# Keytoyze/Mug-Diffusion

Measured on NVIDIA H100. Metric: denoising-steps/sec, higher is better.
Workload: dtype f32

## Files before the change

### include/mugd.h

```cpp
#ifndef MUGD_H
#define MUGD_H

#include <stdint.h>

#ifdef __cplusplus
extern "C" {
#endif

#define MUGD_ABI_VERSION 13

typedef struct mugd_handle mugd_handle;
typedef struct mugd_plan mugd_plan;

enum mugd_status {
    MUGD_OK = 0,
    MUGD_ERR_INVALID = 1,
    MUGD_ERR_CUDA = 2,
    MUGD_ERR_NO_DEVICE = 3,
    MUGD_ERR_OOM = 4
};

enum mugd_op_kind {
    MUGD_OP_GEMM = 1,
    MUGD_OP_GROUPNORM = 2,
// ... 275 lines not shown

int  mugd_remove_mini_jacks(mugd_handle* h, const int32_t* chart_start, int32_t n_charts, double jack_interval,
                            const double* start, const double* end, const uint8_t* is_long, int32_t* x, uint8_t* state,
                            void* workspace, void* stream);

int  mugd_gemm_tc_query(mugd_handle* h, const mugd_gemm* g, int32_t sm_count, int32_t* supported, int32_t* splits,
                        int64_t* workspace_bytes, int32_t* n_tiles);
int  mugd_gemm_tc_variant(const mugd_gemm* g, int32_t sm_count, int32_t* tile_n, int32_t* ctas_per_sm, int32_t* grid_ctas);

int  mugd_set_tc_single_pass_tf32(mugd_handle* h, int enabled);

int  mugd_set_attention_impl(mugd_handle* h, int impl);

int  mugd_set_s4conv_impl(mugd_handle* h, int impl);

int  mugd_debug_set_tc_cost(float kstep128_us, float kstep256_us, float split_us, float two_cta_fixed_us);

int  mugd_debug_set_tc_tile_n(int bn);

int  mugd_debug_set_attention_dump(float* buf);

int  mugd_debug_set_tc_timing(long long* device_buf);

int  mugd_fill_i32(int32_t* dst, int32_t value, void* stream);
int  mugd_abi_sizes(int32_t* out, int32_t n);

#ifdef __cplusplus
}
#endif
#endif
// ... 1 lines not shown
```

### mug_diffusion_b200/csrc/api.cu

```cuda
#include <stdarg.h>
#include <string.h>

#include <vector>

#include "common.cuh"

namespace mugd {

static thread_local char g_err[1024] = "";
bool g_use_pdl = true;

void set_error(const char* fmt, ...) {
    va_list ap;
    va_start(ap, fmt);
    vsnprintf(g_err, sizeof(g_err), fmt, ap);
    va_end(ap);
}

}

struct mugd_handle {
    mugd::DeviceInfo dev;
    int default_gemm_impl = MUGD_GEMM_SIMT;
};
// ... 36 lines not shown
static int run_steps(const mugd_plan* eval_plan, int32_t n_steps, int32_t* step, cudaStream_t st, Before before, After after) {
    mugd_step_advance adv;
    adv.step = step;
    for (int32_t k = 0; k < n_steps; ++k) {
        int rc = before(k);
        if (rc != MUGD_OK) return rc;
        MUGD_CHECK_CUDA(cudaGraphLaunch(eval_plan->exec, st));
        if ((rc = after(k)) != MUGD_OK) return rc;
        if (step && (rc = launch_step_advance(eval_plan->h->dev, adv, st, nullptr)) != MUGD_OK) return rc;
    }
    return MUGD_OK;
}

static int no_kernels(int32_t) { return MUGD_OK; }

template <typename Before>
static int run_tail_steps(const mugd_plan* eval_plan, const mugd_op* tail, int32_t n_tail, int32_t n_steps, cudaStream_t st,
                          Before before) {
    return run_steps(eval_plan, n_steps, nullptr, st, before, [&](int32_t) {
        for (int32_t k = 0; k < n_tail; ++k) {
            int rc = dispatch(eval_plan->h, tail[k], st, nullptr);
            if (rc != MUGD_OK) return rc;
        }
        return (int)MUGD_OK;
    });
}

static int run_dpm_steps(const mugd_plan* eval_plan, const mugd_dpm_ex& e, int32_t n_steps, cudaStream_t st) {
    return run_steps(
        eval_plan, n_steps, e.dpm.step, st, [&](int32_t k) { return e.stage ? launch_stage(*e.stage, k, st) : MUGD_OK; },
// ... 80 lines not shown
}

int mugd_set_attention_impl(mugd_handle* h, int impl) {
    MUGD_REQUIRE(h, "null handle");
    h->dev.attention_impl = impl ? 1 : 0;
    return MUGD_OK;
}

int mugd_set_s4conv_impl(mugd_handle* h, int impl) {
    MUGD_REQUIRE(h, "null handle");
    MUGD_REQUIRE(impl >= 0 && impl <= 2, "set_s4conv_impl: %d (0 = automatic, 1 = resident, 2 = streamed)", impl);
    h->dev.s4conv_impl = impl;
    return MUGD_OK;
}

int mugd_set_pdl(int enabled) {
    g_use_pdl = enabled != 0;
    return MUGD_OK;
}

int mugd_op_run(mugd_handle* h, const mugd_op* op, void* stream) {
    MUGD_REQUIRE(h && op, "mugd_op_run: null argument");
    return dispatch(h, *op, (cudaStream_t)stream, nullptr);
}

int mugd_plan_create(mugd_handle* h, const mugd_op* ops, int32_t n_ops, mugd_plan** out) {
    MUGD_REQUIRE(h && ops && out && n_ops > 0, "mugd_plan_create: bad arguments");
    mugd_plan* p = new mugd_plan();
    p->h = h;
    p->ops.assign(ops, ops + n_ops);
    *out = p;
    return MUGD_OK;
}

int mugd_plan_run(mugd_plan* p, void* stream) {
    MUGD_REQUIRE(p, "null plan");
    int launches = 0;
    const size_t n = p->ops.size();
    std::vector<const mugd_gemm*> next_tc(n, nullptr);
    for (size_t i = n; i-- > 1;) {
        const mugd_op& o = p->ops[i];
        next_tc[i - 1] = o.kind == MUGD_OP_GEMM && gemm_runs_tc(o.u.gemm, p->h->default_gemm_impl) ? &o.u.gemm : next_tc[i];
    }
    for (size_t i = 0; i < n; ++i) {
        int rc = dispatch(p->h, p->ops[i], (cudaStream_t)stream, &launches, next_tc[i]);
        if (rc != MUGD_OK) {
            char prev[900];
            strncpy(prev, g_err, sizeof(prev) - 1);
            prev[sizeof(prev) - 1] = 0;
            set_error("plan op %zu (kind %d, tag %d): %s", i, p->ops[i].kind, p->ops[i].tag, prev);
            return rc;
        }
    }
    p->launches = launches;
    return MUGD_OK;
}

int mugd_plan_capture(mugd_plan* p, void* stream) {
    MUGD_REQUIRE(p, "null plan");
    cudaStream_t st = (cudaStream_t)stream;
// ... 161 lines not shown
```

### mug_diffusion_b200/csrc/common.cuh

```cuda
#pragma once
#include <cuda_runtime.h>
#include <stdint.h>
#include <stdio.h>
#include <string.h>
#include <string>
#include <utility>

#include "../../include/mugd.h"

#if defined(__CUDA_ARCH__) && (__CUDA_ARCH__ != 900)
#error "libmugd is written for sm_90a (H100) only"
#endif

namespace mugd {

void set_error(const char* fmt, ...);

#define MUGD_CHECK_CUDA(expr)                                                             \
    do {                                                                                  \
        cudaError_t _e = (expr);                                                          \
        if (_e != cudaSuccess) {                                                          \
            ::mugd::set_error("%s:%d %s -> %s", __FILE__, __LINE__, #expr,                \
                              cudaGetErrorString(_e));                                    \
            return MUGD_ERR_CUDA;                                                         \
// ... 4 lines not shown
    do {                                                                                  \
        if (!(cond)) {                                                                    \
            ::mugd::set_error(__VA_ARGS__);                                               \
            return MUGD_ERR_INVALID;                                                      \
        }                                                                                 \
    } while (0)

struct DeviceInfo {
    int device = 0;
    int sm_count = 132;
    int cc_major = 0, cc_minor = 0;
    int max_smem_optin = 0;
    int tc_single_pass = 0;
    int attention_impl = 1;
    int s4conv_impl = 0;
};

int launch_gemm(const DeviceInfo& dev, const mugd_gemm& g, int default_impl, const mugd_gemm* next, cudaStream_t st, int* launches);
bool gemm_runs_tc(const mugd_gemm& g, int default_impl);
int launch_groupnorm(const DeviceInfo& dev, const mugd_groupnorm& g, cudaStream_t st, int* launches);
int launch_layernorm(const DeviceInfo& dev, const mugd_layernorm& g, cudaStream_t st, int* launches);
int launch_attention(const DeviceInfo& dev, const mugd_attention& a, cudaStream_t st, int* launches);
int launch_s4conv(const DeviceInfo& dev, const mugd_s4conv& s, cudaStream_t st, int* launches);
int launch_ddim_update(const DeviceInfo& dev, const mugd_ddim_update& d, cudaStream_t st, int* launches);
int launch_transpose(const DeviceInfo& dev, const mugd_transpose& t, cudaStream_t st, int* launches);
int launch_copy2d(const DeviceInfo& dev, const mugd_copy2d& c, cudaStream_t st, int* launches);
int launch_step_advance(const DeviceInfo& dev, const mugd_step_advance& a, cudaStream_t st, int* launches);
int launch_notes(const DeviceInfo& dev, const mugd_notes& n, cudaStream_t st, int* launches);
int launch_embed(const DeviceInfo& dev, const mugd_embed& e, cudaStream_t st, int* launches);
int launch_tf32_split(const DeviceInfo& dev, const mugd_tf32_split& s, cudaStream_t st, int* launches);
int launch_posterior(const DeviceInfo& dev, const mugd_posterior& p, cudaStream_t st, int* launches);
int check_stage(const mugd_stage& s, int32_t n_steps);
int launch_stage(const mugd_stage& s, int32_t i, cudaStream_t st);
int check_plms(const mugd_plms& p);
int launch_plms_combine(const mugd_plms& p, int32_t step, int heun, cudaStream_t st);
int check_ddpm(const mugd_ddpm& d);
int launch_ddpm_update(const mugd_ddpm& d, int32_t k, cudaStream_t st);
int check_dpm(const mugd_dpm& d);
int launch_dpm_update(const mugd_dpm& d, cudaStream_t st);
int check_dpm_ex(const mugd_dpm_ex& e, int32_t n_steps);
int launch_dpm_ex_update(const mugd_dpm_ex& e, cudaStream_t st);
int check_join(const mugd_join& j);
int launch_join(const mugd_join& j, const int32_t* step, cudaStream_t st);
int launch_gemm_tc(const DeviceInfo& dev, const mugd_gemm& g, const mugd_gemm* next, cudaStream_t st, int* launches);
bool gemm_tc_supported(const mugd_gemm& g);

inline int check_cfg(const char* who, int cfg) {
    MUGD_REQUIRE(cfg == 0 || cfg == 1, "%s: cfg=%d", who, cfg);
    return MUGD_OK;
}
inline int check_scale(const char* who, float scale) {
    MUGD_REQUIRE(isfinite(scale), "%s: scale is not finite", who);
    return MUGD_OK;
}
inline int check_x_dup(const char* who, const float* x_dup, int cfg) {
    MUGD_REQUIRE(!x_dup == !cfg, "%s: x_dup must be given exactly when cfg = 1 (the evaluation reads x in both halves)", who);
    return MUGD_OK;
}
inline int check_tile_grid(const char* who, int32_t B, int32_t C, int32_t L) {
// ... 74 lines not shown
```

### mug_diffusion_b200/csrc/gemm_simt.cu

```cuda
#include "common.cuh"

namespace mugd {

constexpr int SG_THREADS = 256;
constexpr int SG_BK = 16;

struct GemmParams {
    mugd_gemm g;
    int nk;
};

__device__ __forceinline__ int conv_src_row(int mode, int l, int t, int Lin, int Lout, int tap_shift, int dil) {
    if (mode == MUGD_CONV_NONE) return l;
    if (mode == MUGD_CONV_SAME) {
        const int r = l + t - 1;
        return (r >= 0 && r < Lin) ? r : -1;
    }
    if (mode == MUGD_CONV_DOWN) {
        const int r = 2 * l + t;
        return (r < Lin) ? r : -1;
    }
    if (mode == MUGD_CONV_TAPS) {
        const int r = l + (t + tap_shift) * dil;
        return (r >= 0 && r < Lin) ? r : -1;
// ... 192 lines not shown
    MUGD_REQUIRE(aligned16(g.A) && aligned16(g.W) && g.lda % 4 == 0 && g.lda >= g.K, "gemm: A/W alignment or lda");
    MUGD_REQUIRE(!g.bias || aligned16(g.bias), "gemm: bias alignment");
    MUGD_REQUIRE(!g.rowvec || (aligned16(g.rowvec) && g.rowvec_b_stride % 4 == 0 && g.rowvec_step_stride % 4 == 0), "gemm: rowvec alignment");
    const int nout = g.gate == MUGD_GATE_NONE ? g.N : g.N / 2;
    const int al = g.gate == MUGD_GATE_NONE ? 4 : 2;
    MUGD_REQUIRE(g.ldc >= nout && g.ldc % al == 0 && (reinterpret_cast<uintptr_t>(g.C) % (4 * al)) == 0, "gemm: C alignment/ldc");
    MUGD_REQUIRE(!g.residual || (g.ldr >= nout && g.ldr % al == 0 && (reinterpret_cast<uintptr_t>(g.residual) % (4 * al)) == 0), "gemm: residual alignment/ldr");
    MUGD_REQUIRE(g.act >= 0 && g.act <= 2 && g.gate >= 0 && g.gate <= 2, "gemm: bad act/gate");
    return MUGD_OK;
}

bool gemm_runs_tc(const mugd_gemm& g, int default_impl) {
    return (g.impl == MUGD_GEMM_AUTO ? default_impl : g.impl) == MUGD_GEMM_TC && gemm_tc_supported(g);
}

int launch_gemm(const DeviceInfo& dev, const mugd_gemm& g, int default_impl, const mugd_gemm* next, cudaStream_t st, int* launches) {
    int rc = validate_gemm(g);
    if (rc != MUGD_OK) return rc;
    int impl = g.impl == MUGD_GEMM_AUTO ? default_impl : g.impl;
    if (impl == MUGD_GEMM_TC) {
        if (gemm_tc_supported(g)) return launch_gemm_tc(dev, g, next, st, launches);
        MUGD_REQUIRE(g.impl != MUGD_GEMM_TC, "gemm: tensor-core path requested but shape unsupported (M=%d N=%d K=%d)", g.M, g.N, g.K);
    }
    MUGD_REQUIRE(!(g.W_hi && g.W_hi == g.W), "gemm: W was split into TF32 hi/lo in place, the FFMA kernel needs the plain fp32 weight (M=%d N=%d K=%d)", g.M, g.N, g.K);
    MUGD_REQUIRE(!g.row_moments && !g.ln_stats,
                 "gemm: the row-moment sink / folded LayerNorm exist on the tensor-core path only (M=%d N=%d K=%d fell to the FFMA kernel)", g.M, g.N, g.K);
    GemmParams p;
    p.g = g;
    p.nk = (g.taps * g.K + g.K2) / SG_BK;
    const long tiles128 = (long)((g.M + 127) / 128) * ((g.N + 127) / 128);
    if (tiles128 >= 2L * dev.sm_count) {
        dim3 grid((g.N + 127) / 128, (g.M + 127) / 128);
        MUGD_CHECK_CUDA(launch_k(gemm_simt_kernel<2, 2>, grid, dim3(SG_THREADS), 0, st, p));
    } else {
        dim3 grid((g.N + 63) / 64, (g.M + 63) / 64);
        MUGD_CHECK_CUDA(launch_k(gemm_simt_kernel<1, 1>, grid, dim3(SG_THREADS), 0, st, p));
// ... 8 lines not shown
```

### mug_diffusion_b200/csrc/gemm_tc.cu

```cuda
#include "gemm_tc.cuh"

namespace mugd {

template <int BN, int EPI>
__global__ void __launch_bounds__(TC_THREADS, 1)
gemm_tc_kernel(const __grid_constant__ CUtensorMap tmA, const __grid_constant__ CUtensorMap tmA1,
               const __grid_constant__ CUtensorMap tmA2, const __grid_constant__ CUtensorMap tmB, const __grid_constant__ CUtensorMap tmWhi,
               const __grid_constant__ CUtensorMap tmWlo, const __grid_constant__ TcParams p) {
    extern __shared__ uint8_t smem_raw[];
    const uint32_t base = (smem_u32(smem_raw) + 1023u) & ~1023u;
    const TcBars<BN> B(base);
    TC_STAMP(p, 0, blockIdx.x == 0 && blockIdx.y == 0 && blockIdx.z == 0);
    if (threadIdx.x < 32) {
        B.init_parallel((int)threadIdx.x);
    } else if (threadIdx.x < 38) {
        const CUtensorMap* m = threadIdx.x == 32 ? &tmA : threadIdx.x == 33 ? &tmA1 : threadIdx.x == 34 ? &tmA2
                             : threadIdx.x == 35 ? &tmB : threadIdx.x == 36 ? &tmWhi : &tmWlo;
        asm volatile("prefetch.tensormap [%0];" ::"l"(reinterpret_cast<uint64_t>(m)) : "memory");
    }
    __syncthreads();
    TC_STAMP(p, 1, blockIdx.x == 0 && blockIdx.y == 0 && blockIdx.z == 0);
    gemm_tc_tile<BN, EPI>(&tmA, &tmA1, &tmA2, &tmB, &tmWhi, &tmWlo, p, blockIdx.x, blockIdx.y, blockIdx.z, base);
}

// ... 140 lines not shown
    p.ws = (float*)g.workspace;
    p.gy = t.gy;
    p.ln_invK = 1.0 / (double)g.K;
    if (next) {
        p.pf_hi = next->W_hi;
        p.pf_lo = p.hot.single_pass ? nullptr : next->W_lo;
        p.pf_bytes = (int64_t)next->N * ((int64_t)next->taps * next->K + next->K2) * 4;
    }
#ifdef MUGD_TC_TIMELINE
    p.dbg = g_tc_dbg;
#endif
    out->BN = t.BN;
    return MUGD_OK;
}

template <int BN, int EPI>
static int tc_launch(const TcPlanned& pl, cudaStream_t st) {
    const TcParams& p = pl.p;
    const TcParams::Hot& h = p.hot;
    if (h.splits > 1) {
        MUGD_CHECK_CUDA(launch_k(gemm_tc_kernel<BN, TC_E_NONE>, dim3(h.gx, p.gy, h.splits), dim3(TC_THREADS), TcSmem<BN>::TOTAL, st, pl.maps[0],
                                 pl.maps[1], pl.maps[2], pl.maps[3], pl.maps[4], pl.maps[5], p));
        MUGD_CHECK_CUDA(launch_k(gemm_tc_reduce_kernel<BN, EPI>, dim3((unsigned)(h.gx * p.gy * (TC_BM / TC_RED_ROWS<BN>))), dim3(TC_THREADS), 0,
                                 st, p));
        return MUGD_OK;
    }
    MUGD_CHECK_CUDA(launch_k(gemm_tc_kernel<BN, EPI>, dim3(h.gx, p.gy, 1), dim3(TC_THREADS), TcSmem<BN>::TOTAL, st, pl.maps[0], pl.maps[1],
                             pl.maps[2], pl.maps[3], pl.maps[4], pl.maps[5], p));
    return MUGD_OK;
}

template <int BN, int... EPI>
static cudaError_t allow_smem_bn(int bytes, std::integer_sequence<int, EPI...>) {
    return allow_dynamic_smem(bytes, gemm_tc_kernel<BN, EPI>...);
}
cudaError_t gemm_tc_allow_smem(int bytes) {
    const cudaError_t e = allow_smem_bn<64>(bytes, std::make_integer_sequence<int, TC_E_COUNT>{});
// ... 2 lines not shown

template <int BN>
static int tc_launch_bn(const TcPlanned& pl, cudaStream_t st) {
    switch (tc_epi_of(pl.p.g)) {
        case TC_E_GEGLU: return tc_launch<BN, TC_E_GEGLU>(pl, st);
        case TC_E_GLU: return tc_launch<BN, TC_E_GLU>(pl, st);
        case TC_E_SILU: return tc_launch<BN, TC_E_SILU>(pl, st);
        case TC_E_GELU: return tc_launch<BN, TC_E_GELU>(pl, st);
        case TC_E_SINK: return tc_launch<BN, TC_E_SINK>(pl, st);
        case TC_E_LN: return tc_launch<BN, TC_E_LN>(pl, st);
        case TC_E_LN_GEGLU: return tc_launch<BN, TC_E_LN_GEGLU>(pl, st);
        default: return tc_launch<BN, TC_E_NONE>(pl, st);
    }
}

int launch_gemm_tc(const DeviceInfo& dev, const mugd_gemm& g, const mugd_gemm* next, cudaStream_t st, int* launches) {
    TcPlanned pl;
    int rc = tc_plan(dev, g, next, &pl);
    if (rc != MUGD_OK) return rc;
    if (pl.BN == 128) rc = tc_launch_bn<128>(pl, st);
    else rc = tc_launch_bn<64>(pl, st);
    if (rc != MUGD_OK) return rc;
    if (launches) *launches += pl.p.hot.splits > 1 ? 2 : 1;
    return MUGD_OK;
}

}

extern "C" int mugd_debug_set_tc_cost(float kstep128_us, float kstep256_us, float split_us, float two_cta_fixed_us) {
    (void)kstep256_us;
    (void)two_cta_fixed_us;
    if (kstep128_us > 0.f) mugd::g_tc_kstep128 = kstep128_us;
    if (split_us > 0.f) mugd::g_tc_split = split_us;
    return MUGD_OK;
// ... 54 lines not shown
```

### mug_diffusion_b200/csrc/gemm_tc.cuh

```cuda
#pragma once
#include <cuda.h>
#include <stddef.h>

#include <type_traits>

#include "common.cuh"
#include "wgmma.cuh"

namespace mugd {

constexpr int TC_BM = 128;
constexpr int TC_BK = 32;
constexpr int TC_THREADS = 256;
constexpr uint32_t TC_A_BYTES = TC_BM * TC_BK * 4;

struct TcParams {
    struct Hot {
        int32_t Lrows, Bs;
        int32_t box_l, box_b;
        int32_t tiles_per_sample;
        int32_t it_base, it_rem;
        int32_t it_main;
        int32_t kblocks;
        int32_t total_it;
        int32_t splits;
        int32_t single_pass;
        int32_t conv_mode, tap_shift, tap_dilation;
        int32_t gx;
    } hot;
    mugd_gemm g;
    float* ws;
    int32_t gy;
    double ln_invK;
    const float* pf_hi;
    const float* pf_lo;
    int64_t pf_bytes;
#ifdef MUGD_TC_TIMELINE
    long long* dbg;
#endif
};
static_assert(sizeof(TcParams::Hot) == 64 && offsetof(TcParams, hot) == 0, "the hot fields are the first 64 bytes of the parameters");

#ifdef __CUDACC__
__device__ __forceinline__ long long gtimer() {
    long long t;
    asm volatile("mov.u64 %0, %%globaltimer;" : "=l"(t) :: "memory");
    return t;
}
#ifdef MUGD_TC_TIMELINE
#define TC_STAMP(p, k, cta0) do { if ((p).dbg && (cta0) && threadIdx.x == 0) (p).dbg[k] = gtimer(); } while (0)
#else
// ... 151 lines not shown
}

__device__ __forceinline__ void tc_tile_rows(const TcParams& p, int by, int& b_base, int& l_base, int& rows_valid) {
    const TcParams::Hot& h = p.hot;
    if (h.Lrows >= TC_BM) {
        b_base = by / h.tiles_per_sample;
        l_base = (by % h.tiles_per_sample) * TC_BM;
        rows_valid = min(TC_BM, h.Lrows - l_base);
    } else {
        b_base = by * h.box_b;
        l_base = 0;
        rows_valid = min(h.box_b, h.Bs - b_base) * h.Lrows;
    }
}

template <int BN>
struct TcBars {
    using S = TcSmem<BN>;
    static constexpr int COUNT = 2 * S::STAGES;
    static_assert(8 * COUNT <= (int)S::BAR_BYTES, "barrier block");
    uint32_t bars;
    __device__ __forceinline__ explicit TcBars(uint32_t base) : bars(base + S::TILE_BYTES) {}
    __device__ __forceinline__ uint32_t full(int s) const { return bars + 8u * s; }
    __device__ __forceinline__ uint32_t empty(int s) const { return bars + 8u * (S::STAGES + s); }
    __device__ __forceinline__ void init_parallel(int t) const {
        if (t >= COUNT) return;
        mbar_init(bars + 8u * t, t < S::STAGES ? 1u : (uint32_t)(TC_THREADS / 32));
        mbar_init_fence();
    }
};
// ... 172 lines not shown
    __syncthreads();
    TC_STAMP(p, 3, bx == 0 && by == 0 && bz == 0);
    {
        const float* rowvec = g.rowvec ? g.rowvec + (int64_t)epi_step * g.rowvec_step_stride : nullptr;
        if (h.splits > 1) {
            const int tile_lin = by * h.gx + bx;
            float* wsp = p.ws + ((int64_t)tile_lin * h.splits + bz) * (TC_BM * BN);
            constexpr int C4 = BN / 4;
            constexpr int U = 8;
#pragma unroll 1
            for (int i0 = 0; i0 < TC_BM * C4; i0 += TC_THREADS * U) {
                float4 a4[U];
#pragma unroll
                for (int u = 0; u < U; ++u) {
                    const int idx = i0 + u * TC_THREADS + (int)threadIdx.x;
                    const int row = idx / C4, c4 = idx - row * C4;
                    a4[u] = lds_f4(base + (uint32_t)(row * SP + c4 * 4) * 4u);
                }
#pragma unroll
                for (int u = 0; u < U; ++u) st_f4(wsp + (i0 + u * TC_THREADS + (int)threadIdx.x) * 4, a4[u]);
            }
        } else {
            using E = TcEpiTraits<EPI>;
            tc_store_tile<BN, E::ACT, E::GATE, E::MODE>(g, base, m_base, n0, rows_valid, rowvec, base + S::TILE_BYTES - 1024u, epi_bias, epi_cs);
        }
    }
    TC_STAMP(p, 4, bx == 0 && by == 0 && bz == 0);
}

template <int BN> constexpr int TC_RED_ROWS = TC_THREADS / (BN / 4);

// ... 73 lines not shown
```

### mug_diffusion_b200/csrc/norm.cu

```cuda
#include "common.cuh"

namespace mugd {

constexpr int GN_THREADS = 256;
constexpr int GN_MAXV = 32;

__device__ __forceinline__ void gn_block_stats(double s, double ss, double inv_n, float eps, float& mean, float& rstd) {
    __shared__ double red[2][GN_THREADS / 32];
    s = warp_sum(s);
    ss = warp_sum(ss);
    const int warp = threadIdx.x >> 5, lane = threadIdx.x & 31;
    if (lane == 0) { red[0][warp] = s; red[1][warp] = ss; }
    __syncthreads();
    double ts = 0.0, tss = 0.0;
#pragma unroll
    for (int w = 0; w < GN_THREADS / 32; ++w) { ts += red[0][w]; tss += red[1][w]; }
    const double m = ts * inv_n;
    const double var = tss * inv_n - m * m;
    const float v = fmaxf((float)var, 0.f) + eps;
    float r = rsqrtf(v);
    r = r * (1.5f - 0.5f * v * r * r);
    mean = (float)m;
    rstd = r;
}

template <int NV>
__global__ void __launch_bounds__(GN_THREADS)
groupnorm_silu_reg_kernel(const float* __restrict__ x, int64_t ldx, float* __restrict__ y, int64_t ldy,
                          const float* __restrict__ gamma, const float* __restrict__ beta,
                          int L, int C, int G, float eps, int silu) {
    pdl_wait();
    const int g = blockIdx.x, b = blockIdx.y;
    const int cg = C / G;
    const int q = cg >> 2;
    const int total = L * q;
    const double inv_n = 1.0 / ((double)L * cg);
    const float* xb = x + (int64_t)b * L * ldx + (int64_t)g * cg;
    float* yb = y + (int64_t)b * L * ldy + (int64_t)g * cg;
    float4 v[NV];
#pragma unroll
    for (int u = 0; u < NV; ++u) {
        const int i = (int)threadIdx.x + u * GN_THREADS;
        v[u] = make_float4(0.f, 0.f, 0.f, 0.f);
        if (i < total) {
            const int row = i / q, qq = i - row * q;
            v[u] = ld_f4(xb + (int64_t)row * ldx + qq * 4);
        }
    }
    double s = 0.0, ss = 0.0;
#pragma unroll
    for (int u = 0; u < NV; ++u) {
        s += (double)v[u].x + (double)v[u].y + (double)v[u].z + (double)v[u].w;
        ss += (double)v[u].x * v[u].x + (double)v[u].y * v[u].y + (double)v[u].z * v[u].z + (double)v[u].w * v[u].w;
    }
    const float* gm = gamma + g * cg;
    const float* bt = beta + g * cg;
    constexpr bool PRE = NV <= 8;
    float4 gav[PRE ? NV : 1], bev[PRE ? NV : 1];
    if constexpr (PRE) {
#pragma unroll
        for (int u = 0; u < NV; ++u) {
            const int i = (int)threadIdx.x + u * GN_THREADS;
            const int qq = i < total ? i % q : 0;
            gav[u] = ld_f4(gm + qq * 4);
            bev[u] = ld_f4(bt + qq * 4);
        }
    }
    float mean, rstd;
    gn_block_stats(s, ss, inv_n, eps, mean, rstd);
#pragma unroll
    for (int u = 0; u < NV; ++u) {
        const int i = (int)threadIdx.x + u * GN_THREADS;
        if (i < total) {
            const int row = i / q, qq = i - row * q;
            float4 ga, be;
            if constexpr (PRE) { ga = gav[u]; be = bev[u]; }
            else { ga = ld_f4(gm + qq * 4); be = ld_f4(bt + qq * 4); }
            float4 o;
            o.x = (v[u].x - mean) * rstd * ga.x + be.x;
            o.y = (v[u].y - mean) * rstd * ga.y + be.y;
            o.z = (v[u].z - mean) * rstd * ga.z + be.z;
            o.w = (v[u].w - mean) * rstd * ga.w + be.w;
            if (silu) { o.x = silu_f(o.x); o.y = silu_f(o.y); o.z = silu_f(o.z); o.w = silu_f(o.w); }
            st_f4(yb + (int64_t)row * ldy + qq * 4, o);
        }
    }
}

__global__ void __launch_bounds__(GN_THREADS)
groupnorm_silu_kernel(const float* __restrict__ x, int64_t ldx, float* __restrict__ y, int64_t ldy,
                      const float* __restrict__ gamma, const float* __restrict__ beta,
                      int L, int C, int G, float eps, int silu) {
    pdl_wait();
    const int g = blockIdx.x, b = blockIdx.y;
    const int cg = C / G;
    const int q = cg >> 2;
    const int total = L * q;
    const double inv_n = 1.0 / ((double)L * cg);
    const float* xb = x + (int64_t)b * L * ldx + (int64_t)g * cg;
    float* yb = y + (int64_t)b * L * ldy + (int64_t)g * cg;

// ... 11 lines not shown
    for (int i = threadIdx.x; i < total; i += GN_THREADS) {
        const int row = i / q, qq = i - row * q;
        const float4 v = ld_f4(xb + (int64_t)row * ldx + qq * 4);
        const float4 ga = ld_f4(gm + qq * 4);
        const float4 be = ld_f4(bt + qq * 4);
        float4 o;
        o.x = (v.x - mean) * rstd * ga.x + be.x;
        o.y = (v.y - mean) * rstd * ga.y + be.y;
        o.z = (v.z - mean) * rstd * ga.z + be.z;
        o.w = (v.w - mean) * rstd * ga.w + be.w;
        if (silu) { o.x = silu_f(o.x); o.y = silu_f(o.y); o.z = silu_f(o.z); o.w = silu_f(o.w); }
        st_f4(yb + (int64_t)row * ldy + qq * 4, o);
    }
}

int launch_groupnorm(const DeviceInfo&, const mugd_groupnorm& g, cudaStream_t st, int* launches) {
    MUGD_REQUIRE(g.B > 0 && g.L > 0 && g.C > 0 && g.G > 0, "groupnorm: empty shape B=%d L=%d C=%d G=%d", g.B, g.L, g.C, g.G);
    MUGD_REQUIRE(g.C % g.G == 0 && (g.C / g.G) % 4 == 0, "groupnorm: C/G must be a multiple of 4 (C=%d G=%d)", g.C, g.G);
    MUGD_REQUIRE(g.ldx % 4 == 0 && g.ldy % 4 == 0 && aligned16(g.x) && aligned16(g.y) && aligned16(g.gamma) && aligned16(g.beta),
                 "groupnorm: operands must be 16-byte aligned with ld %% 4 == 0");
    MUGD_REQUIRE(g.ldx >= g.C && g.ldy >= g.C, "groupnorm: leading dimension smaller than C");
    dim3 grid(g.G, g.B);
    const int per_thread = (g.L * (g.C / g.G / 4) + GN_THREADS - 1) / GN_THREADS;
#define GN_GO(K) MUGD_CHECK_CUDA(launch_k(K, grid, dim3(GN_THREADS), 0, st, g.x, g.ldx, g.y, g.ldy, g.gamma, g.beta, g.L, g.C, g.G, g.eps, g.silu))
    if (per_thread <= 2) GN_GO(groupnorm_silu_reg_kernel<2>);
    else if (per_thread <= 4) GN_GO(groupnorm_silu_reg_kernel<4>);
    else if (per_thread <= 8) GN_GO(groupnorm_silu_reg_kernel<8>);
    else if (per_thread <= 16) GN_GO(groupnorm_silu_reg_kernel<16>);
    else if (per_thread <= GN_MAXV) GN_GO(groupnorm_silu_reg_kernel<GN_MAXV>);
    else GN_GO(groupnorm_silu_kernel);
#undef GN_GO
    if (launches) *launches += 1;
    return MUGD_OK;
}

constexpr int LN_WARPS = 8;
constexpr int LN_MAXQ = 8;

// ... 62 lines not shown
```

### mug_diffusion_b200/lib.py

```python
from __future__ import annotations

import ctypes as C
import os
from typing import Optional

HERE = os.path.dirname(os.path.abspath(__file__))
LIB_PATH = os.environ.get("MUGD_LIB") or os.path.join(HERE, "libmugd.so")

(OP_GEMM, OP_GROUPNORM, OP_LAYERNORM, OP_ATTENTION, OP_S4CONV, OP_DDIM_UPDATE, OP_TRANSPOSE, OP_COPY2D, OP_STEP_ADVANCE, OP_NOTES, OP_EMBED,
 OP_TF32_SPLIT, OP_POSTERIOR) = range(1, 14)
CONV_NONE, CONV_SAME, CONV_DOWN, CONV_UP, CONV_TAPS = range(5)
ACT_NONE, ACT_SILU, ACT_GELU = range(3)
GATE_NONE, GATE_GEGLU, GATE_GLU = range(3)
GEMM_AUTO, GEMM_SIMT, GEMM_TC = range(3)
ABI_VERSION = 13

_f = C.c_void_p


class Gemm(C.Structure):
    _fields_ = [("A", _f), ("lda", C.c_int64), ("W", _f), ("W_hi", _f), ("W_lo", _f), ("bias", _f), ("rowvec", _f),
                ("rowvec_b_stride", C.c_int64), ("rowvec_step_stride", C.c_int64), ("step", _f),
                ("residual", _f), ("ldr", C.c_int64), ("C", _f), ("ldc", C.c_int64),
                ("M", C.c_int32), ("N", C.c_int32), ("K", C.c_int32),
# ... 186 lines not shown
    lib.mugd_sample_plms.argtypes = [C.c_void_p, C.POINTER(Plms), C.c_int32, C.c_int32, C.c_void_p]
    lib.mugd_plms_combine.argtypes = [C.POINTER(Plms), C.c_int32, C.c_int32, C.c_void_p]
    lib.mugd_sample_ddpm.argtypes = [C.c_void_p, C.POINTER(Ddpm), C.c_int32, C.c_int32, C.c_void_p]
    lib.mugd_ddpm_update.argtypes = [C.POINTER(Ddpm), C.c_void_p]
    lib.mugd_sample_dpm.argtypes = [C.c_void_p, C.POINTER(Dpm), C.c_int32, C.c_int32, C.c_void_p]
    lib.mugd_dpm_update.argtypes = [C.POINTER(Dpm), C.c_void_p]
    lib.mugd_sample_dpm_ex.argtypes = [C.c_void_p, C.POINTER(DpmEx), C.c_int32, C.c_int32, C.c_void_p]
    lib.mugd_dpm_ex_update.argtypes = [C.POINTER(DpmEx), C.c_void_p]
    lib.mugd_stochastic_encode.argtypes = [C.POINTER(QEncode), C.c_void_p]
    lib.mugd_sample_join.argtypes = [C.c_void_p, C.POINTER(Join), C.POINTER(Op), C.c_int32, C.c_int32, C.c_int32, C.c_void_p]
    lib.mugd_plan_save.argtypes = [C.c_void_p, C.POINTER(Region), C.c_int32, C.c_char_p]
    lib.mugd_plan_load.argtypes = [C.c_void_p, C.c_char_p, C.POINTER(Region), C.c_int32, C.POINTER(C.c_void_p)]
    lib.mugd_set_tc_single_pass_tf32.argtypes = [C.c_void_p, C.c_int]
    lib.mugd_set_attention_impl.argtypes = [C.c_void_p, C.c_int]
    lib.mugd_set_s4conv_impl.argtypes = [C.c_void_p, C.c_int]
    lib.mugd_debug_set_tc_tile_n.argtypes = [C.c_int]
    lib.mugd_debug_set_tc_cost.argtypes = [C.c_float, C.c_float, C.c_float, C.c_float]
    if os.environ.get("MUGD_TC_COST"):
        lib.mugd_debug_set_tc_cost(*([float(v) for v in os.environ["MUGD_TC_COST"].split(",")] + [0.0] * 4)[:4])
    if os.environ.get("MUGD_TC_TILE"):
        lib.mugd_debug_set_tc_tile_n(int(os.environ["MUGD_TC_TILE"]))
    if os.environ.get("MUGD_TC_BN"):
        lib.mugd_debug_set_tc_tile_n(int(os.environ["MUGD_TC_BN"]))
    if os.environ.get("MUGD_PDL") in ("0", "1"):
        lib.mugd_set_pdl(int(os.environ["MUGD_PDL"]))
    _lib = lib
    return lib


def check(rc: int, what: str = ""):
    if rc != 0:
        msg = load().mugd_last_error().decode(errors="replace")
        if rc == 4:
            import torch
            raise torch.cuda.OutOfMemoryError(f"{what}: {msg}")
        raise MugdError(f"{what} failed (status {rc}): {msg}")


EXPORTED_SYMBOLS = [
    "mugd_abi_version", "mugd_last_error", "mugd_create", "mugd_destroy", "mugd_device_info", "mugd_set_gemm_impl",
    "mugd_op_run", "mugd_plan_create", "mugd_plan_run", "mugd_plan_capture", "mugd_plan_replay",
    "mugd_plan_launch_count", "mugd_plan_destroy", "mugd_s4_kernel_gen", "mugd_fill_i32", "mugd_abi_sizes", "mugd_gemm_tc_query",
    "mugd_set_pdl", "mugd_set_tc_single_pass_tf32", "mugd_set_attention_impl", "mugd_set_s4conv_impl", "mugd_debug_set_tc_tile_n", "mugd_debug_set_tc_cost", "mugd_gemm_tc_variant",
    "mugd_debug_set_attention_dump", "mugd_debug_set_tc_timing", "mugd_sample", "mugd_plan_save", "mugd_plan_load", "mugd_plan_regions", "mugd_plan_ops",
    "mugd_melspec", "mugd_grid_scan", "mugd_chart_snap", "mugd_remove_mini_jacks",
    "mugd_sample_staged", "mugd_sample_plms", "mugd_plms_combine",
    "mugd_sample_ddpm", "mugd_ddpm_update", "mugd_stochastic_encode", "mugd_sample_join",
    "mugd_sample_dpm", "mugd_dpm_update", "mugd_sample_dpm_ex", "mugd_dpm_ex_update",
]
```

Before: 244.0.

## Fuse split-K GEMM reduction into following GroupNorm kernel

When a split-K tensor-core GEMM with a plain epilogue is immediately followed by a GroupNorm over its output, the GEMM now launches only its partial-product kernel. The GroupNorm kernel then sums the split-K partials from the workspace, applies the GEMM finish (bias, residual, row vector, store of C) and normalizes in the same pass. This drops one kernel launch and one write-then-read round trip of the GEMM output per matched pair. The workspace layout switches to quad-major for these pairs so the GroupNorm reads line up. The cost is per-group blocks that each reduce many splits, which can leave the GPU with lower parallelism than the dedicated reduce kernel had. The path is on by default and can be disabled.

Result: faster. 248.1, median of 6 (+1.7%).

```diff
diff --git a/include/mugd.h b/include/mugd.h
--- a/include/mugd.h
+++ b/include/mugd.h
@@ -313,6 +313,9 @@
 
 int  mugd_set_s4conv_impl(mugd_handle* h, int impl);
 
+int  mugd_set_gn_reduce_fusion(mugd_handle* h, int enabled);
+int  mugd_gn_reduce_pairs(const mugd_op* ops, int32_t n_ops, int32_t sm_count, int32_t* paired, int32_t* n_pairs);
+
 int  mugd_debug_set_tc_cost(float kstep128_us, float kstep256_us, float split_us, float two_cta_fixed_us);
 
 int  mugd_debug_set_tc_tile_n(int bn);
diff --git a/mug_diffusion_b200/csrc/api.cu b/mug_diffusion_b200/csrc/api.cu
--- a/mug_diffusion_b200/csrc/api.cu
+++ b/mug_diffusion_b200/csrc/api.cu
@@ -4,6 +4,7 @@
 #include <vector>
 
 #include "common.cuh"
+#include "gemm_tc.cuh"
 
 namespace mugd {
 
@@ -74,6 +75,11 @@
 
 static int no_kernels(int32_t) { return MUGD_OK; }
 
+static bool gn_finishes_op(const mugd_op* op, size_t n, int default_impl, int sm_count) {
+    return n >= 2 && op[0].kind == MUGD_OP_GEMM && op[1].kind == MUGD_OP_GROUPNORM &&
+           gn_finishes_gemm(op[0].u.gemm, op[1].u.gn, default_impl, sm_count);
+}
+
 template <typename Before>
 static int run_tail_steps(const mugd_plan* eval_plan, const mugd_op* tail, int32_t n_tail, int32_t n_steps, cudaStream_t st,
                           Before before) {
@@ -184,6 +190,30 @@
     return MUGD_OK;
 }
 
+int mugd_set_gn_reduce_fusion(mugd_handle* h, int enabled) {
+    MUGD_REQUIRE(h, "null handle");
+    MUGD_REQUIRE(enabled == 0 || enabled == 1, "set_gn_reduce_fusion: %d (0 = reduce launch, 1 = the GroupNorm finishes the GEMM)", enabled);
+    h->dev.gn_reduce_fusion = enabled;
+    return MUGD_OK;
+}
+
+int mugd_gn_reduce_pairs(const mugd_op* ops, int32_t n_ops, int32_t sm_count, int32_t* paired, int32_t* n_pairs) {
+    MUGD_REQUIRE(ops && n_ops > 0, "gn_reduce_pairs: bad arguments");
+    const int sms = sm_count > 0 ? sm_count : 132;
+    int32_t count = 0;
+    for (int32_t i = 0; i < n_ops; ++i) {
+        const bool pair = gn_finishes_op(ops + i, (size_t)(n_ops - i), MUGD_GEMM_TC, sms);
+        if (paired) paired[i] = pair ? 1 : 0;
+        if (pair) {
+            ++count;
+            if (paired) paired[i + 1] = 0;
+            ++i;
+        }
+    }
+    if (n_pairs) *n_pairs = count;
+    return MUGD_OK;
+}
+
 int mugd_set_pdl(int enabled) {
     g_use_pdl = enabled != 0;
     return MUGD_OK;
@@ -207,13 +237,22 @@
     MUGD_REQUIRE(p, "null plan");
     int launches = 0;
     const size_t n = p->ops.size();
+    const mugd_handle* h = p->h;
     std::vector<const mugd_gemm*> next_tc(n, nullptr);
     for (size_t i = n; i-- > 1;) {
         const mugd_op& o = p->ops[i];
-        next_tc[i - 1] = o.kind == MUGD_OP_GEMM && gemm_runs_tc(o.u.gemm, p->h->default_gemm_impl) ? &o.u.gemm : next_tc[i];
-    }
+        next_tc[i - 1] = o.kind == MUGD_OP_GEMM && gemm_runs_tc(o.u.gemm, h->default_gemm_impl) ? &o.u.gemm : next_tc[i];
+    }
+    const cudaStream_t st = (cudaStream_t)stream;
     for (size_t i = 0; i < n; ++i) {
-        int rc = dispatch(p->h, p->ops[i], (cudaStream_t)stream, &launches, next_tc[i]);
+        int rc;
+        if (h->dev.gn_reduce_fusion && gn_finishes_op(p->ops.data() + i, n - i, h->default_gemm_impl, h->dev.sm_count)) {
+            TcPlanned pl;
+            rc = launch_gemm(h->dev, p->ops[i].u.gemm, h->default_gemm_impl, next_tc[i], st, &launches, &pl);
+            if (rc == MUGD_OK) rc = launch_groupnorm(h->dev, p->ops[++i].u.gn, st, &launches, &pl);
+        } else {
+            rc = dispatch(p->h, p->ops[i], st, &launches, next_tc[i]);
+        }
         if (rc != MUGD_OK) {
             char prev[900];
             strncpy(prev, g_err, sizeof(prev) - 1);
diff --git a/mug_diffusion_b200/csrc/common.cuh b/mug_diffusion_b200/csrc/common.cuh
--- a/mug_diffusion_b200/csrc/common.cuh
+++ b/mug_diffusion_b200/csrc/common.cuh
@@ -42,11 +42,16 @@
     int tc_single_pass = 0;
     int attention_impl = 1;
     int s4conv_impl = 0;
+    int gn_reduce_fusion = 1;
 };
 
-int launch_gemm(const DeviceInfo& dev, const mugd_gemm& g, int default_impl, const mugd_gemm* next, cudaStream_t st, int* launches);
+struct TcPlanned;
+
+int launch_gemm(const DeviceInfo& dev, const mugd_gemm& g, int default_impl, const mugd_gemm* next, cudaStream_t st, int* launches,
+                TcPlanned* partials = nullptr);
 bool gemm_runs_tc(const mugd_gemm& g, int default_impl);
-int launch_groupnorm(const DeviceInfo& dev, const mugd_groupnorm& g, cudaStream_t st, int* launches);
+bool gn_finishes_gemm(const mugd_gemm& g, const mugd_groupnorm& n, int default_impl, int sm_count);
+int launch_groupnorm(const DeviceInfo& dev, const mugd_groupnorm& g, cudaStream_t st, int* launches, const TcPlanned* partials = nullptr);
 int launch_layernorm(const DeviceInfo& dev, const mugd_layernorm& g, cudaStream_t st, int* launches);
 int launch_attention(const DeviceInfo& dev, const mugd_attention& a, cudaStream_t st, int* launches);
 int launch_s4conv(const DeviceInfo& dev, const mugd_s4conv& s, cudaStream_t st, int* launches);
@@ -70,7 +75,7 @@
 int launch_dpm_ex_update(const mugd_dpm_ex& e, cudaStream_t st);
 int check_join(const mugd_join& j);
 int launch_join(const mugd_join& j, const int32_t* step, cudaStream_t st);
-int launch_gemm_tc(const DeviceInfo& dev, const mugd_gemm& g, const mugd_gemm* next, cudaStream_t st, int* launches);
+int launch_gemm_tc(const DeviceInfo& dev, const mugd_gemm& g, const mugd_gemm* next, cudaStream_t st, int* launches, TcPlanned* partials);
 bool gemm_tc_supported(const mugd_gemm& g);
 
 inline int check_cfg(const char* who, int cfg) {
diff --git a/mug_diffusion_b200/csrc/gemm_simt.cu b/mug_diffusion_b200/csrc/gemm_simt.cu
--- a/mug_diffusion_b200/csrc/gemm_simt.cu
+++ b/mug_diffusion_b200/csrc/gemm_simt.cu
@@ -230,12 +230,14 @@
     return (g.impl == MUGD_GEMM_AUTO ? default_impl : g.impl) == MUGD_GEMM_TC && gemm_tc_supported(g);
 }
 
-int launch_gemm(const DeviceInfo& dev, const mugd_gemm& g, int default_impl, const mugd_gemm* next, cudaStream_t st, int* launches) {
+int launch_gemm(const DeviceInfo& dev, const mugd_gemm& g, int default_impl, const mugd_gemm* next, cudaStream_t st, int* launches,
+                TcPlanned* partials) {
     int rc = validate_gemm(g);
     if (rc != MUGD_OK) return rc;
     int impl = g.impl == MUGD_GEMM_AUTO ? default_impl : g.impl;
+    MUGD_REQUIRE(!partials || (impl == MUGD_GEMM_TC && gemm_tc_supported(g)), "gemm: only the tensor-core kernel can leave split-K partials");
     if (impl == MUGD_GEMM_TC) {
-        if (gemm_tc_supported(g)) return launch_gemm_tc(dev, g, next, st, launches);
+        if (gemm_tc_supported(g)) return launch_gemm_tc(dev, g, next, st, launches, partials);
         MUGD_REQUIRE(g.impl != MUGD_GEMM_TC, "gemm: tensor-core path requested but shape unsupported (M=%d N=%d K=%d)", g.M, g.N, g.K);
     }
     MUGD_REQUIRE(!(g.W_hi && g.W_hi == g.W), "gemm: W was split into TF32 hi/lo in place, the FFMA kernel needs the plain fp32 weight (M=%d N=%d K=%d)", g.M, g.N, g.K);
diff --git a/mug_diffusion_b200/csrc/gemm_tc.cu b/mug_diffusion_b200/csrc/gemm_tc.cu
--- a/mug_diffusion_b200/csrc/gemm_tc.cu
+++ b/mug_diffusion_b200/csrc/gemm_tc.cu
@@ -178,13 +178,21 @@
     return MUGD_OK;
 }
 
+template <int BN>
+static int tc_launch_partials(const TcPlanned& pl, cudaStream_t st) {
+    const TcParams& p = pl.p;
+    MUGD_CHECK_CUDA(launch_k(gemm_tc_kernel<BN, TC_E_NONE>, dim3(p.hot.gx, p.gy, p.hot.splits), dim3(TC_THREADS), TcSmem<BN>::TOTAL, st,
+                             pl.maps[0], pl.maps[1], pl.maps[2], pl.maps[3], pl.maps[4], pl.maps[5], p));
+    return MUGD_OK;
+}
+
 template <int BN, int EPI>
 static int tc_launch(const TcPlanned& pl, cudaStream_t st) {
     const TcParams& p = pl.p;
     const TcParams::Hot& h = p.hot;
     if (h.splits > 1) {
-        MUGD_CHECK_CUDA(launch_k(gemm_tc_kernel<BN, TC_E_NONE>, dim3(h.gx, p.gy, h.splits), dim3(TC_THREADS), TcSmem<BN>::TOTAL, st, pl.maps[0],
-                                 pl.maps[1], pl.maps[2], pl.maps[3], pl.maps[4], pl.maps[5], p));
+        int rc = tc_launch_partials<BN>(pl, st);
+        if (rc != MUGD_OK) return rc;
         MUGD_CHECK_CUDA(launch_k(gemm_tc_reduce_kernel<BN, EPI>, dim3((unsigned)(h.gx * p.gy * (TC_BM / TC_RED_ROWS<BN>))), dim3(TC_THREADS), 0,
                                  st, p));
         return MUGD_OK;
@@ -217,10 +225,19 @@
     }
 }
 
-int launch_gemm_tc(const DeviceInfo& dev, const mugd_gemm& g, const mugd_gemm* next, cudaStream_t st, int* launches) {
-    TcPlanned pl;
+int launch_gemm_tc(const DeviceInfo& dev, const mugd_gemm& g, const mugd_gemm* next, cudaStream_t st, int* launches, TcPlanned* partials) {
+    TcPlanned local;
+    TcPlanned& pl = partials ? *partials : local;
     int rc = tc_plan(dev, g, next, &pl);
     if (rc != MUGD_OK) return rc;
+    if (partials) {
+        MUGD_REQUIRE(pl.p.hot.splits > 1 && tc_epi_of(g) == TC_E_NONE, "gemm_tc: only a split-K GEMM with a plain epilogue can leave its partials");
+        pl.p.ws_quad_major = 1;
+        rc = pl.BN == 128 ? tc_launch_partials<128>(pl, st) : tc_launch_partials<64>(pl, st);
+        if (rc != MUGD_OK) return rc;
+        if (launches) *launches += 1;
+        return MUGD_OK;
+    }
     if (pl.BN == 128) rc = tc_launch_bn<128>(pl, st);
     else rc = tc_launch_bn<64>(pl, st);
     if (rc != MUGD_OK) return rc;
diff --git a/mug_diffusion_b200/csrc/gemm_tc.cuh b/mug_diffusion_b200/csrc/gemm_tc.cuh
--- a/mug_diffusion_b200/csrc/gemm_tc.cuh
+++ b/mug_diffusion_b200/csrc/gemm_tc.cuh
@@ -35,6 +35,7 @@
     const float* pf_hi;
     const float* pf_lo;
     int64_t pf_bytes;
+    int32_t ws_quad_major;
 #ifdef MUGD_TC_TIMELINE
     long long* dbg;
 #endif
@@ -216,6 +217,17 @@
     }
 }
 
+__device__ __forceinline__ int64_t tc_ws_offset(const TcParams& p, int bn, int m, int n) {
+    const TcParams::Hot& h = p.hot;
+    const int s = m / h.Lrows, l = m - s * h.Lrows;
+    int by, r;
+    if (h.Lrows >= TC_BM) { by = s * h.tiles_per_sample + l / TC_BM; r = l % TC_BM; }
+    else { by = s / h.box_b; r = m - by * h.box_b * h.Lrows; }
+    const int bx = n / bn, c = n - bx * bn;
+    const int64_t in_tile = p.ws_quad_major ? (int64_t)(c >> 2) * (TC_BM * 4) + r * 4 + (c & 3) : (int64_t)r * bn + c;
+    return ((int64_t)(by * h.gx + bx) * h.splits) * (TC_BM * bn) + in_tile;
+}
+
 template <int BN>
 struct TcBars {
     using S = TcSmem<BN>;
@@ -418,7 +430,9 @@
 #pragma unroll
                 for (int u = 0; u < U; ++u) {
                     const int idx = i0 + u * TC_THREADS + (int)threadIdx.x;
-                    const int row = idx / C4, c4 = idx - row * C4;
+                    int row, c4;
+                    if (p.ws_quad_major) { c4 = idx / TC_BM; row = idx - c4 * TC_BM; }
+                    else { row = idx / C4; c4 = idx - row * C4; }
                     a4[u] = lds_f4(base + (uint32_t)(row * SP + c4 * 4) * 4u);
                 }
 #pragma unroll
diff --git a/mug_diffusion_b200/csrc/norm.cu b/mug_diffusion_b200/csrc/norm.cu
--- a/mug_diffusion_b200/csrc/norm.cu
+++ b/mug_diffusion_b200/csrc/norm.cu
@@ -1,9 +1,11 @@
 #include "common.cuh"
+#include "gemm_tc.cuh"
 
 namespace mugd {
 
 constexpr int GN_THREADS = 256;
 constexpr int GN_MAXV = 32;
+constexpr int GN_REDUCE_MAXV = 2;
 
 __device__ __forceinline__ void gn_block_stats(double s, double ss, double inv_n, float eps, float& mean, float& rstd) {
     __shared__ double red[2][GN_THREADS / 32];
@@ -22,6 +24,47 @@
     r = r * (1.5f - 0.5f * v * r * r);
     mean = (float)m;
     rstd = r;
+}
+
+template <int NV>
+__device__ __forceinline__ void gn_normalize_slab(const float4 (&v)[NV], float* yb, int64_t ldy, const float* gm, const float* bt, int q,
+                                                  int total, double inv_n, float eps, int silu) {
+    double s = 0.0, ss = 0.0;
+#pragma unroll
+    for (int u = 0; u < NV; ++u) {
+        s += (double)v[u].x + (double)v[u].y + (double)v[u].z + (double)v[u].w;
+        ss += (double)v[u].x * v[u].x + (double)v[u].y * v[u].y + (double)v[u].z * v[u].z + (double)v[u].w * v[u].w;
+    }
+    constexpr bool PRE = NV <= 8;
+    float4 gav[PRE ? NV : 1], bev[PRE ? NV : 1];
+    if constexpr (PRE) {
+#pragma unroll
+        for (int u = 0; u < NV; ++u) {
+            const int i = (int)threadIdx.x + u * GN_THREADS;
+            const int qq = i < total ? i % q : 0;
+            gav[u] = ld_f4(gm + qq * 4);
+            bev[u] = ld_f4(bt + qq * 4);
+        }
+    }
+    float mean, rstd;
+    gn_block_stats(s, ss, inv_n, eps, mean, rstd);
+#pragma unroll
+    for (int u = 0; u < NV; ++u) {
+        const int i = (int)threadIdx.x + u * GN_THREADS;
+        if (i < total) {
+            const int row = i / q, qq = i - row * q;
+            float4 ga, be;
+            if constexpr (PRE) { ga = gav[u]; be = bev[u]; }
+            else { ga = ld_f4(gm + qq * 4); be = ld_f4(bt + qq * 4); }
+            float4 o;
+            o.x = (v[u].x - mean) * rstd * ga.x + be.x;
+            o.y = (v[u].y - mean) * rstd * ga.y + be.y;
+            o.z = (v[u].z - mean) * rstd * ga.z + be.z;
+            o.w = (v[u].w - mean) * rstd * ga.w + be.w;
+            if (silu) { o.x = silu_f(o.x); o.y = silu_f(o.y); o.z = silu_f(o.z); o.w = silu_f(o.w); }
+            st_f4(yb + (int64_t)row * ldy + qq * 4, o);
+        }
+    }
 }
 
 template <int NV>
@@ -36,7 +79,6 @@
     const int total = L * q;
     const double inv_n = 1.0 / ((double)L * cg);
     const float* xb = x + (int64_t)b * L * ldx + (int64_t)g * cg;
-    float* yb = y + (int64_t)b * L * ldy + (int64_t)g * cg;
     float4 v[NV];
 #pragma unroll
     for (int u = 0; u < NV; ++u) {
@@ -47,44 +89,79 @@
             v[u] = ld_f4(xb + (int64_t)row * ldx + qq * 4);
         }
     }
-    double s = 0.0, ss = 0.0;
-#pragma unroll
-    for (int u = 0; u < NV; ++u) {
-        s += (double)v[u].x + (double)v[u].y + (double)v[u].z + (double)v[u].w;
-        ss += (double)v[u].x * v[u].x + (double)v[u].y * v[u].y + (double)v[u].z * v[u].z + (double)v[u].w * v[u].w;
-    }
-    const float* gm = gamma + g * cg;
-    const float* bt = beta + g * cg;
-    constexpr bool PRE = NV <= 8;
-    float4 gav[PRE ? NV : 1], bev[PRE ? NV : 1];
-    if constexpr (PRE) {
-#pragma unroll
-        for (int u = 0; u < NV; ++u) {
-            const int i = (int)threadIdx.x + u * GN_THREADS;
-            const int qq = i < total ? i % q : 0;
-            gav[u] = ld_f4(gm + qq * 4);
-            bev[u] = ld_f4(bt + qq * 4);
-        }
-    }
-    float mean, rstd;
-    gn_block_stats(s, ss, inv_n, eps, mean, rstd);
+    gn_normalize_slab<NV>(v, y + (int64_t)b * L * ldy + (int64_t)g * cg, ldy, gamma + g * cg, beta + g * cg, q, total, inv_n, eps, silu);
+}
+
+template <int NV>
+__global__ void __launch_bounds__(GN_THREADS)
+groupnorm_reduce_kernel(const __grid_constant__ TcParams p, int bn, float* __restrict__ y, int64_t ldy, const float* __restrict__ gamma,
+                        const float* __restrict__ beta, int L, int C, int G, float eps, int silu) {
+    static_assert(NV <= GN_REDUCE_MAXV, "bias, residual and row-vector quads of every float4 are held in registers");
+    constexpr int ZU = 8;
+    const mugd_gemm& gg = p.g;
+    const int g = blockIdx.x, b = blockIdx.y;
+    const int cg = C / G;
+    const int q = cg >> 2;
+    const int total = L * q;
+    const double inv_n = 1.0 / ((double)L * cg);
+    const int splits = p.hot.splits;
+    float4 bia[NV], res[NV], rvv[NV];
+    const int step = gg.step ? *gg.step : 0;
+    const float* rowvec = gg.rowvec ? gg.rowvec + (int64_t)step * gg.rowvec_step_stride : nullptr;
+#pragma unroll
+    for (int u = 0; u < NV; ++u) {
+        const int i = (int)threadIdx.x + u * GN_THREADS;
+        const int row = i < total ? i / q : 0, qq = i - row * q;
+        const int m = b * L + row, n = g * cg + qq * 4;
+        bia[u] = res[u] = rvv[u] = make_float4(0.f, 0.f, 0.f, 0.f);
+        if (i < total && gg.bias) bia[u] = ld_f4(gg.bias + n);
+        if (i < total && gg.residual) res[u] = ld_f4(gg.residual + (int64_t)m * gg.ldr + n);
+        if (i < total && rowvec) rvv[u] = ld_f4(rowvec + (int64_t)(m / gg.Lout) * gg.rowvec_b_stride + n);
+    }
+    pdl_wait();
+    const float* src[NV];
+    float4 t4[NV][ZU];
+#pragma unroll
+    for (int u = 0; u < NV; ++u) {
+        const int i = (int)threadIdx.x + u * GN_THREADS;
+        const int row = i < total ? i / q : 0, qq = i - row * q;
+        src[u] = p.ws + tc_ws_offset(p, bn, b * L + row, g * cg + qq * 4);
+#pragma unroll
+        for (int k = 0; k < ZU; ++k) {
+            t4[u][k] = make_float4(0.f, 0.f, 0.f, 0.f);
+            if (i < total && k < splits) t4[u][k] = __ldcg(reinterpret_cast<const float4*>(src[u] + (int64_t)k * (TC_BM * bn)));
+        }
+    }
+    float4 v[NV];
+#pragma unroll
+    for (int u = 0; u < NV; ++u) {
+        const int i = (int)threadIdx.x + u * GN_THREADS;
+        float4 acc = make_float4(0.f, 0.f, 0.f, 0.f);
+#pragma unroll
+        for (int k = 0; k < ZU; ++k) { acc.x += t4[u][k].x; acc.y += t4[u][k].y; acc.z += t4[u][k].z; acc.w += t4[u][k].w; }
+        for (int z0 = ZU; z0 < splits; z0 += ZU) {
+            float4 t[ZU];
+#pragma unroll
+            for (int k = 0; k < ZU; ++k) {
+                t[k] = make_float4(0.f, 0.f, 0.f, 0.f);
+                if (i < total && z0 + k < splits) t[k] = __ldcg(reinterpret_cast<const float4*>(src[u] + (int64_t)(z0 + k) * (TC_BM * bn)));
+            }
+#pragma unroll
+            for (int k = 0; k < ZU; ++k) { acc.x += t[k].x; acc.y += t[k].y; acc.z += t[k].z; acc.w += t[k].w; }
+        }
+        v[u] = acc;
+    }
 #pragma unroll
     for (int u = 0; u < NV; ++u) {
         const int i = (int)threadIdx.x + u * GN_THREADS;
         if (i < total) {
             const int row = i / q, qq = i - row * q;
-            float4 ga, be;
-            if constexpr (PRE) { ga = gav[u]; be = bev[u]; }
-            else { ga = ld_f4(gm + qq * 4); be = ld_f4(bt + qq * 4); }
-            float4 o;
-            o.x = (v[u].x - mean) * rstd * ga.x + be.x;
-            o.y = (v[u].y - mean) * rstd * ga.y + be.y;
-            o.z = (v[u].z - mean) * rstd * ga.z + be.z;
-            o.w = (v[u].w - mean) * rstd * ga.w + be.w;
-            if (silu) { o.x = silu_f(o.x); o.y = silu_f(o.y); o.z = silu_f(o.z); o.w = silu_f(o.w); }
-            st_f4(yb + (int64_t)row * ldy + qq * 4, o);
-        }
-    }
+            const int m = b * L + row, n = g * cg + qq * 4;
+            v[u] = tc_finish4<MUGD_ACT_NONE, MUGD_GATE_NONE, false>(gg, gg.C + (int64_t)m * gg.ldc + n, v[u], bia[u], rvv[u], res[u],
+                                                                    make_float4(0.f, 0.f, 0.f, 0.f), make_float2(0.f, 1.f), m, n);
+        }
+    }
+    gn_normalize_slab<NV>(v, y + (int64_t)b * L * ldy + (int64_t)g * cg, ldy, gamma + g * cg, beta + g * cg, q, total, inv_n, eps, silu);
 }
 
 __global__ void __launch_bounds__(GN_THREADS)
@@ -126,14 +203,34 @@
     }
 }
 
-int launch_groupnorm(const DeviceInfo&, const mugd_groupnorm& g, cudaStream_t st, int* launches) {
+static int gn_per_thread(const mugd_groupnorm& g) { return (g.L * (g.C / g.G / 4) + GN_THREADS - 1) / GN_THREADS; }
+
+bool gn_finishes_gemm(const mugd_gemm& g, const mugd_groupnorm& n, int default_impl, int sm_count) {
+    if (!gemm_runs_tc(g, default_impl) || tc_epi_of(g) != TC_E_NONE) return false;
+    if (n.x != g.C || n.ldx != g.ldc || (int64_t)n.B * n.L != g.M || n.C != g.N) return false;
+    if (n.G <= 0 || n.C % n.G != 0 || (n.C / n.G) % 4 != 0 || gn_per_thread(n) > GN_REDUCE_MAXV) return false;
+    return tc_geometry(g, sm_count, g.split_k).hot.splits > 2;
+}
+
+int launch_groupnorm(const DeviceInfo&, const mugd_groupnorm& g, cudaStream_t st, int* launches, const TcPlanned* partials) {
     MUGD_REQUIRE(g.B > 0 && g.L > 0 && g.C > 0 && g.G > 0, "groupnorm: empty shape B=%d L=%d C=%d G=%d", g.B, g.L, g.C, g.G);
     MUGD_REQUIRE(g.C % g.G == 0 && (g.C / g.G) % 4 == 0, "groupnorm: C/G must be a multiple of 4 (C=%d G=%d)", g.C, g.G);
     MUGD_REQUIRE(g.ldx % 4 == 0 && g.ldy % 4 == 0 && aligned16(g.x) && aligned16(g.y) && aligned16(g.gamma) && aligned16(g.beta),
                  "groupnorm: operands must be 16-byte aligned with ld %% 4 == 0");
     MUGD_REQUIRE(g.ldx >= g.C && g.ldy >= g.C, "groupnorm: leading dimension smaller than C");
     dim3 grid(g.G, g.B);
-    const int per_thread = (g.L * (g.C / g.G / 4) + GN_THREADS - 1) / GN_THREADS;
+    const int per_thread = gn_per_thread(g);
+    if (partials) {
+        const TcParams& p = partials->p;
+        MUGD_REQUIRE(g.x == p.g.C && g.ldx == p.g.ldc && (int64_t)g.B * g.L == p.g.M && g.C == p.g.N && p.hot.splits > 1 &&
+                         per_thread <= GN_REDUCE_MAXV,
+                     "groupnorm: cannot finish this GEMM (x must be its split-K output, at most %d float4 per thread)", GN_REDUCE_MAXV);
+#define GN_RED(K) MUGD_CHECK_CUDA(launch_k(K, grid, dim3(GN_THREADS), 0, st, p, partials->BN, g.y, g.ldy, g.gamma, g.beta, g.L, g.C, g.G, g.eps, g.silu))
+        GN_RED(groupnorm_reduce_kernel<GN_REDUCE_MAXV>);
+#undef GN_RED
+        if (launches) *launches += 1;
+        return MUGD_OK;
+    }
 #define GN_GO(K) MUGD_CHECK_CUDA(launch_k(K, grid, dim3(GN_THREADS), 0, st, g.x, g.ldx, g.y, g.ldy, g.gamma, g.beta, g.L, g.C, g.G, g.eps, g.silu))
     if (per_thread <= 2) GN_GO(groupnorm_silu_reg_kernel<2>);
     else if (per_thread <= 4) GN_GO(groupnorm_silu_reg_kernel<4>);
diff --git a/mug_diffusion_b200/lib.py b/mug_diffusion_b200/lib.py
--- a/mug_diffusion_b200/lib.py
+++ b/mug_diffusion_b200/lib.py
@@ -224,6 +224,8 @@
     lib.mugd_set_tc_single_pass_tf32.argtypes = [C.c_void_p, C.c_int]
     lib.mugd_set_attention_impl.argtypes = [C.c_void_p, C.c_int]
     lib.mugd_set_s4conv_impl.argtypes = [C.c_void_p, C.c_int]
+    lib.mugd_set_gn_reduce_fusion.argtypes = [C.c_void_p, C.c_int]
+    lib.mugd_gn_reduce_pairs.argtypes = [C.POINTER(Op), C.c_int32, C.c_int32, C.POINTER(C.c_int32), C.POINTER(C.c_int32)]
     lib.mugd_debug_set_tc_tile_n.argtypes = [C.c_int]
     lib.mugd_debug_set_tc_cost.argtypes = [C.c_float, C.c_float, C.c_float, C.c_float]
     if os.environ.get("MUGD_TC_COST"):
@@ -251,7 +253,7 @@
     "mugd_abi_version", "mugd_last_error", "mugd_create", "mugd_destroy", "mugd_device_info", "mugd_set_gemm_impl",
     "mugd_op_run", "mugd_plan_create", "mugd_plan_run", "mugd_plan_capture", "mugd_plan_replay",
     "mugd_plan_launch_count", "mugd_plan_destroy", "mugd_s4_kernel_gen", "mugd_fill_i32", "mugd_abi_sizes", "mugd_gemm_tc_query",
-    "mugd_set_pdl", "mugd_set_tc_single_pass_tf32", "mugd_set_attention_impl", "mugd_set_s4conv_impl", "mugd_debug_set_tc_tile_n", "mugd_debug_set_tc_cost", "mugd_gemm_tc_variant",
+    "mugd_set_pdl", "mugd_set_tc_single_pass_tf32", "mugd_set_attention_impl", "mugd_set_s4conv_impl", "mugd_set_gn_reduce_fusion", "mugd_gn_reduce_pairs", "mugd_debug_set_tc_tile_n", "mugd_debug_set_tc_cost", "mugd_gemm_tc_variant",
     "mugd_debug_set_attention_dump", "mugd_debug_set_tc_timing", "mugd_sample", "mugd_plan_save", "mugd_plan_load", "mugd_plan_regions", "mugd_plan_ops",
     "mugd_melspec", "mugd_grid_scan", "mugd_chart_snap", "mugd_remove_mini_jacks",
     "mugd_sample_staged", "mugd_sample_plms", "mugd_plms_combine",
```
